# thalesfm/differentiable-renderer

Measured on AMD Instinct MI355X. Metric: Mray/s (fwd+bwd), Cornell 512x512 @64spp depth 8, higher is better.
Workload: dtype f32; 1 GPU; config 3: Cornell 512x512, 64 spp, depth 8, fwd + radiative backprop w.r.t. the albedos; scene 'cornell' (cornell box of render.cpp:26-59) 512x512, 64 spp per GPU, depth 8 (-b 8 -p 1), fwd + radiative-backprop gradients of 4 parameters; program=builtin, parallelism=1 GPU, gpu_max_hw_queues=4 (set by this script before the HIP runtime started)

## Files before the change

### differentiable-renderer_amd/csrc/drt_path.h

```cpp
#pragma once

#include "drt_kernels.h"

#define DRT_DRAW_TABLE (3 * DRT_MAX_DEPTH + 8)

struct PathArgs {
    int32_t W, H, spp;
    int32_t shard, n_shards, band;
    uint32_t Pb, p0, Sb, s0, spr, n_ranges, n_groups;
    int32_t min_bounces, depth_cap, cap_is_roulette, cap_draws;
    uint32_t rr_threshold, seed, rng_stream;
    uint32_t regen_min;
    uint32_t shade_min, descend_min;
    int32_t gimg_param;
    uint32_t gen_rows, gen_clog2;
    uint32_t hist_lds, hist_stride;
    uint32_t gimg_row, pad_gen;
    unsigned long long hist_ovf;
    double p_rr, inv_p_rr;
    double eye[3], fwd[3], right[3], up[3];
    double tan_half, aspect, inv_W, inv_H;
    float p_rr_f, inv_p_rr_f;
    float eye_f[3], fwd_f[3], right_f[3], up_f[3], cs_step_f, ct_step_f;
};

__device__ inline uint32_t path_global_pixel(const PathArgs& a, uint32_t lp)
{
    uint32_t ly = lp / (uint32_t)a.W, x = lp - ly * (uint32_t)a.W;
    uint32_t y = ly;
    if (a.n_shards > 1) {
        uint32_t b = ly / (uint32_t)a.band, r = ly - b * (uint32_t)a.band;
        y = (b * (uint32_t)a.n_shards + (uint32_t)a.shard) * (uint32_t)a.band + r;
    }
    return y * (uint32_t)a.W + x;
}

template <typename SG>
__device__ inline HitRec<float> path_closest_hit(const DevScene<float>* __restrict__ sc, const ProgRecs<SG::n>& recs, float4 ra, float2 rb)
{
    return closest_hit_prog<SG>(sc, recs, mk<float>(ra.x, ra.y, ra.z), mk<float>(ra.w, rb.x, rb.y));
}
template <typename SG>
__device__ inline HitRec<double> path_closest_hit(const DevScene<double>* __restrict__ sc, const ProgRecs<SG::n, double>& recs, double4 ra, double2 rb)
{
    if (SG::n > 0)
        return closest_hit_sig<SG, double>(recs, mk<double>(ra.x, ra.y, ra.z), mk<double>(ra.w, rb.x, rb.y));
    const double4 ra1[1] = {ra};
    const double2 rb1[1] = {rb};
    HitRec<double> h1[1];
    closest_hit_n<double, 1>(sc, sc->n_shapes, ra1, rb1, h1);
    return h1[0];
}

#define DRT_SIG_CORNELL                                                                                                   \
    ((unsigned long long)DRT_PK_SPHERE | (unsigned long long)DRT_PK_SPHERE << 3 | (unsigned long long)DRT_PK_AX << 6 |    \
     (unsigned long long)DRT_PK_PLANE << 9 | (unsigned long long)DRT_PK_AZ << 12 | (unsigned long long)DRT_PK_AZ << 15 |  \
     (unsigned long long)DRT_PK_AY << 18 | (unsigned long long)DRT_PK_AY << 21 | (unsigned long long)DRT_PK_SPHERE << 24)
#define DRT_NSIG_CORNELL 9
typedef KindSig<DRT_SIG_CORNELL, 0ull, 0ull, 0ull, DRT_NSIG_CORNELL> SigCornell;


template <typename R>
struct PathSceneLds {
    struct {
        int n_shapes, n_materials, n_emitters, n_params;
        DevShape<R> shapes[DRT_MAX_SHAPES];
        DevMaterial<R> materials[DRT_MAX_MATERIALS];
        int emitter_param[DRT_MAX_EMITTERS];
        int flat[DRT_MAX_SHAPES];
    } sc;
    R params[DRT_PATH_LDS_PARAMS * 3];
#ifdef DRT_USER_SHAPES
    R user_q[DRT_MAX_SHAPES][4];
#endif
};

template <typename R, bool ALL_LDS = false>
__device__ inline V3<R> load_param(const PathSceneLds<R>& lds, const R* __restrict__ params, int id)
{
    if (ALL_LDS || id < DRT_PATH_LDS_PARAMS)
        return mk<R>(lds.params[id * 3], lds.params[id * 3 + 1], lds.params[id * 3 + 2]);
    return mk<R>(params[id * 3], params[id * 3 + 1], params[id * 3 + 2]);
}

template <typename R>
__device__ inline void stage_path_scene(PathSceneLds<R>& lds, const DevScene<R>* __restrict__ sc, const R* __restrict__ params)
{
    const int ns = sc->n_shapes, nm = sc->n_materials, ne = sc->n_emitters;
    if (threadIdx.x < 4)
        reinterpret_cast<int*>(&lds.sc)[threadIdx.x] = reinterpret_cast<const int*>(sc)[threadIdx.x];
    {
        const int* src = reinterpret_cast<const int*>(sc->shapes);
        int* dst = reinterpret_cast<int*>(lds.sc.shapes);
        for (int i = threadIdx.x; i < ns * (int)(sizeof(DevShape<R>) / sizeof(int)); i += blockDim.x)
            dst[i] = src[i];
    }
    {
        const int* src = reinterpret_cast<const int*>(sc->materials);
        int* dst = reinterpret_cast<int*>(lds.sc.materials);
        for (int i = threadIdx.x; i < nm * (int)(sizeof(DevMaterial<R>) / sizeof(int)); i += blockDim.x)
            dst[i] = src[i];
    }
    for (int i = threadIdx.x; i < ne; i += blockDim.x)
        lds.sc.emitter_param[i] = sc->emitter_param[i];
    for (int i = threadIdx.x; i < ns; i += blockDim.x)
        lds.sc.flat[i] = sc->flat[i];
#ifdef DRT_USER_SHAPES
    for (int i = threadIdx.x; i < ns * 4; i += blockDim.x)
        lds.user_q[i >> 2][i & 3] = sc->user_q[i >> 2][i & 3];
#endif
    const int np = sc->n_params < DRT_PATH_LDS_PARAMS ? sc->n_params : DRT_PATH_LDS_PARAMS;
    for (int i = threadIdx.x; i < np * 3; i += blockDim.x)
        lds.params[i] = params[i];
    __syncthreads();
}


template <typename R>
struct TangentLds {
    R colnz[DRT_FAST_PARAMS][4];
    R invc[DRT_FAST_PARAMS][4];
    uint32_t inc[DRT_FAST_PARAMS][4];
};

template <typename R, typename SL>
__device__ inline void stage_tangents(TangentLds<R>& tl, const SL& lds)
{
    if (threadIdx.x < DRT_FAST_PARAMS) {
        const int p = threadIdx.x;
        const bool in = p < lds.sc.n_params;
        uint32_t zinc = 0, zbits = 0;
#pragma unroll
        for (int ch = 0; ch < 3; ++ch) {
            const R c = in ? lds.params[p * 3 + ch] : R(1);
            const bool zero = abs_r(c) < R(1e-18);
            tl.colnz[p][ch] = zero ? R(1) : c;
            tl.invc[p][ch] = zero ? R(0) : R(1) / c;
            zinc |= zero ? 1u << (8 * ch) : 0u;
            zbits |= zero ? 1u << ch : 0u;
        }
        tl.colnz[p][3] = R(0);
        tl.invc[p][3] = R(0);
        tl.inc[p][0] = p < 4 ? 1u << (8 * p) : 0u;
        tl.inc[p][1] = p >= 4 ? 1u << (8 * (p - 4)) : 0u;
        tl.inc[p][2] = zinc;
        tl.inc[p][3] = zbits;
    }
    __syncthreads();
}

template <typename R, int NP, int NC>
struct Tangents {
    uint32_t cnt[NC > 4 ? 2 : 1];
    uint32_t zc;
    R* acc;
    __device__ inline V3<R> acc_get(int p) const { return mk<R>(acc[(p * 3) * DRT_BLOCK], acc[(p * 3 + 1) * DRT_BLOCK], acc[(p * 3 + 2) * DRT_BLOCK]); }
    __device__ inline void acc_set(int p, V3<R> v) { acc[(p * 3) * DRT_BLOCK] = v.x; acc[(p * 3 + 1) * DRT_BLOCK] = v.y; acc[(p * 3 + 2) * DRT_BLOCK] = v.z; }
    __device__ inline void new_path() { cnt[0] = 0; if (NC > 4) cnt[NC > 4 ? 1 : 0] = 0; zc = 0; }
};

#define DRT_NP_ANY (-1)
#ifndef DRT_LOCKSTEP_MIN_BLOCKS
#define DRT_LOCKSTEP_MIN_BLOCKS 7
#endif
#ifndef DRT_LOCKSTEP_GEN_MIN_BLOCKS
#define DRT_LOCKSTEP_GEN_MIN_BLOCKS 6
#endif
#ifndef DRT_LOCKSTEP_SPEC_MIN_BLOCKS
#define DRT_LOCKSTEP_SPEC_MIN_BLOCKS 6
#endif
#ifndef DRT_REGEN_MIN_BLOCKS
#define DRT_REGEN_MIN_BLOCKS 5
#endif
#ifndef DRT_F64_MIN_BLOCKS
#define DRT_F64_MIN_BLOCKS 4
#endif
#ifndef DRT_GEN_TABLE
#define DRT_GEN_TABLE 408
#endif
template <bool B, typename X, typename Y> struct PickT { typedef X T; };
template <typename X, typename Y> struct PickT<false, X, Y> { typedef Y T; };
struct NoLds { int unused; };
template <typename R> struct GenAcc { typedef double T; };
#ifdef DRT_GEN_F32
template <> struct GenAcc<float> { typedef float T; };
#endif

template <typename R>
struct GenLds {
    R colnz[DRT_PATH_LDS_PARAMS][4];
    R invc[DRT_PATH_LDS_PARAMS][4];
};

template <typename R, typename SL>
__device__ inline void stage_gen(GenLds<R>& gl, const SL& lds, const DevScene<R>* __restrict__ sc)
{
    for (int p = threadIdx.x; p < DRT_PATH_LDS_PARAMS; p += blockDim.x) {
        const bool in = p < lds.sc.n_params;
        uint32_t zinc = 0, zbits = 0;
#pragma unroll
        for (int ch = 0; ch < 3; ++ch) {
            const R c = in ? lds.params[p * 3 + ch] : R(1);
            const bool zero = abs_r(c) < R(1e-18);
            gl.colnz[p][ch] = zero ? R(1) : c;
            gl.invc[p][ch] = zero ? R(0) : R(1) / c;
            zinc |= zero ? 1u << (8 * ch) : 0u;
            zbits |= zero ? 1u << ch : 0u;
        }
        const uint32_t slot = in ? (uint32_t)sc->grad_slot[p] : DRT_SLOT_NONE;
        gl.colnz[p][3] = pid_pack(R(0), zinc);
        gl.invc[p][3] = pid_pack(R(0), slot | zbits << 16);
    }
    __syncthreads();
}

template <typename R, int NC>
struct Tangents<R, DRT_NP_ANY, NC> {
    typedef typename GenAcc<R>::T GT;
    uint32_t cur;
    uint32_t zc;
    uint32_t nv;
    uint32_t* hist;
    uint32_t* hist_ovf;
    uint32_t hist_lds, hist_stride;
    const GenLds<R>* gl;
    GT* table;
    uint32_t clog2;
    R* acc;
    V3<R> gsum;
    uint32_t gimg_row;
    __device__ inline void new_path() { cur = 0xFFFFFFFFu; zc = 0; nv = 0; }
    __device__ inline void store_word(uint32_t w, uint32_t v)
    {
        if (w < hist_lds) hist[w * DRT_BLOCK] = v;
        else hist_ovf[(size_t)(w - hist_lds) * hist_stride] = v;
    }
    __device__ inline uint32_t load_word(uint32_t w) const
    {
        return w < hist_lds ? hist[w * DRT_BLOCK] : hist_ovf[(size_t)(w - hist_lds) * hist_stride];
    }
    template <bool UNIFORM>
    __device__ inline void push(bool live, uint32_t id)
    {
        const uint32_t shifted = (cur >> 8) | (id << 24);
        if (UNIFORM) {
            cur = shifted;
            ++nv;
            if ((nv & 3u) == 0u) {
                store_word((nv >> 2) - 1u, cur);
                cur = 0xFFFFFFFFu;
            }
        } else {
            cur = live ? shifted : cur;
            nv += live ? 1u : 0u;
            if (live && (nv & 3u) == 0u) {
                store_word((nv >> 2) - 1u, cur);
                cur = 0xFFFFFFFFu;
            }
        }
    }
    __device__ inline void add(uint32_t row, V3<R> v)
    {
        if constexpr (NC == 1) {
            const bool mine = row == gimg_row;
            gsum = mk<R>(gsum.x + (mine ? v.x : R(0)), gsum.y + (mine ? v.y : R(0)), gsum.z + (mine ? v.z : R(0)));
        }
        GT* t = table + ((row * 3u) << clog2);
        atomicAdd(t, (GT)v.x);
        atomicAdd(t + (1u << clog2), (GT)v.y);
        atomicAdd(t + (2u << clog2), (GT)v.z);
    }
    __device__ inline void add_word(uint32_t wd, V3<R> TgE, V3<R> U)
    {
#pragma unroll
        for (int b = 0; b < 4; ++b) {
            const uint32_t id = (wd >> (8 * b)) & 0xFFu;
            const bool valid = id != 0xFFu;
            if (wave_any(valid)) {
                if (valid) {
                    const R* rec = gl->invc[id];
                    const R ix = rec[0], iy = rec[1], iz = rec[2];
                    const uint32_t bits = pid_unpack(rec[3]);
                    const uint32_t row = bits & 0xFFFFu;
                    if (row != DRT_SLOT_NONE)
                        add(row, mk<R>((bits & 0x10000u) ? U.x : TgE.x * ix, (bits & 0x20000u) ? U.y : TgE.y * iy,
                                       (bits & 0x40000u) ? U.z : TgE.z * iz));
                }
            }
        }
    }
};

template <typename R>
struct GenBlock {
    GenLds<R> gl;
    typename GenAcc<R>::T table[DRT_BLOCK / DRT_WAVE][DRT_GEN_TABLE];
};
template <typename R>
__device__ inline void gen_zero(GenBlock<R>& gb)
{
    typedef typename GenAcc<R>::T GT;
    for (uint32_t i = threadIdx.x; i < (DRT_BLOCK / DRT_WAVE) * DRT_GEN_TABLE; i += DRT_BLOCK)
        (&gb.table[0][0])[i] = GT(0);
}
template <typename R, int NC, typename SL>
__device__ inline void gen_begin(GenBlock<R>& gb, const SL& lds, const DevScene<R>* __restrict__ sc, const PathArgs& a, uint32_t* hist,
                                 uint32_t* hist_ovf, Tangents<R, DRT_NP_ANY, NC>& tg)
{
    stage_gen(gb.gl, lds, sc);
    tg.gl = &gb.gl;
    tg.hist = hist + threadIdx.x;
    tg.hist_ovf = hist_ovf + (size_t)blockIdx.x * DRT_BLOCK + threadIdx.x;
    tg.gsum = mk<R>(R(0), R(0), R(0));
    tg.gimg_row = a.gimg_row;
    tg.hist_lds = a.hist_lds;
    tg.hist_stride = a.hist_stride;
    tg.clog2 = a.gen_clog2;
    tg.table = &gb.table[threadIdx.x / DRT_WAVE][threadIdx.x & ((1u << a.gen_clog2) - 1u)];
    tg.acc = nullptr;
    tg.new_path();
}
template <typename R>
__device__ inline void gen_finish(const GenBlock<R>& gb, const PathArgs& a, double* __restrict__ gpart)
{
    __syncthreads();
    const uint32_t copies = 1u << a.gen_clog2;
    for (uint32_t r = threadIdx.x; r < a.gen_rows; r += DRT_BLOCK) {
        double v = 0;
        for (int ww = 0; ww < DRT_BLOCK / DRT_WAVE; ++ww)
            for (uint32_t c = 0; c < copies; ++c)
                v += (double)gb.table[ww][(r << a.gen_clog2) + c];
        gpart[(size_t)blockIdx.x * a.gen_rows + r] = v;
    }
}

template <typename R, int NP, int NC, bool LOSS = false, typename SL = PathSceneLds<R>>
__device__ inline void add_emission(const SL& lds, const TangentLds<R>& tl, const R* __restrict__ params, uint32_t eid, R inv_pk,
                                    V3<R> T, V3<R> g, V3<R>& L, Tangents<R, NP, NC>& tg)
{
    const V3<R> E = load_param<R, (NP != 0)>(lds, params, (int)eid) * inv_pk;
    V3<R> Tr = T;
    if (NC > 0 || NP == DRT_NP_ANY)
        Tr = mk<R>((tg.zc & 0xFFu) ? R(0) : T.x, (tg.zc & 0xFF00u) ? R(0) : T.y, (tg.zc & 0xFF0000u) ? R(0) : T.z);
    L = L + Tr * E;
    if constexpr (NP == DRT_NP_ANY) {
        if (LOSS)
            g = mk<R>(R(2) * (L.x - g.x), R(2) * (L.y - g.y), R(2) * (L.z - g.z));
        const V3<R> gE = g * E;
        const uint32_t ebits = pid_unpack(tg.gl->invc[eid < DRT_PATH_LDS_PARAMS ? eid : 0][3]);
        if ((ebits & 0xFFFFu) != DRT_SLOT_NONE && eid < DRT_PATH_LDS_PARAMS)
            tg.add(ebits & 0xFFFFu, g * Tr * inv_pk);
        const V3<R> TgE = Tr * gE;
        const V3<R> U = mk<R>((tg.zc & 0xFFu) == 0x1u ? T.x * gE.x : R(0), (tg.zc & 0xFF00u) == 0x100u ? T.y * gE.y : R(0),
                              (tg.zc & 0xFF0000u) == 0x10000u ? T.z * gE.z : R(0));
        const uint32_t nw = tg.nv >> 2;
        for (uint32_t w = 0; wave_any(w < nw); ++w)
            tg.add_word(w < nw ? tg.load_word(w) : 0xFFFFFFFFu, TgE, U);
        tg.add_word(tg.cur, TgE, U);
    } else
    if constexpr (NP > 0) {
        if (NC > 0)
            asm volatile("" ::: "memory");
        if (LOSS)
            g = mk<R>(R(2) * (L.x - g.x), R(2) * (L.y - g.y), R(2) * (L.z - g.z));
        const V3<R> gE = g * E, gT = g * Tr * inv_pk;
#pragma unroll
        for (int p = 0; p < NP; ++p) {
            const bool own = eid == (uint32_t)p;
            const V3<R> ap = tg.acc_get(p);
            const V3<R> a0 = mk<R>(ap.x + (own ? gT.x : R(0)), ap.y + (own ? gT.y : R(0)), ap.z + (own ? gT.z : R(0)));
            if (p < NC) {
                const uint32_t n = (tg.cnt[p >> 2] >> (8 * (p & 3))) & 0xFFu;
                const R nf = (R)(int)n;
                V3<R> dT = mk<R>(Tr.x * (nf * tl.invc[p][0]), Tr.y * (nf * tl.invc[p][1]), Tr.z * (nf * tl.invc[p][2]));
                const uint32_t zb = __builtin_amdgcn_readfirstlane(tl.inc[p][3]);
                if (zb) {
                    const bool one = n == 1u;
                    if (zb & 1u) dT.x = (one && (tg.zc & 0xFFu) == 0x1u) ? T.x : R(0);
                    if (zb & 2u) dT.y = (one && (tg.zc & 0xFF00u) == 0x100u) ? T.y : R(0);
                    if (zb & 4u) dT.z = (one && (tg.zc & 0xFF0000u) == 0x10000u) ? T.z : R(0);
                }
                tg.acc_set(p, mk<R>(fma_r(dT.x, gE.x, a0.x), fma_r(dT.y, gE.y, a0.y), fma_r(dT.z, gE.z, a0.z)));
            } else
                tg.acc_set(p, a0);
        }
    }
}

template <typename R>
struct CameraLane {
    R cs0, ct0;
};

template <typename R>
struct PathVertex {
    V3<R> P, nrm, d;
    uint32_t ids;
    int material;
    bool hit, scattered;
};

template <typename R, bool SPEC, int NP, int NC, typename SG>
__device__ inline void path_bounce(const PathArgs& a, const PathSceneLds<R>& lds, const TangentLds<R>& tl, const DevScene<R>* __restrict__ sc,
                                   const R* __restrict__ params, const ProgRecs<SG::n, R>& recs, uint32_t key,
                                   R pk, R inv_pk, uint32_t n_theta, bool next_rr, bool next_cap, bool live, V3<R> g,
                                   typename Q4<R>::T& ra, typename Q2<R>::T& rb, V3<R>& T, V3<R>& L, Tangents<R, NP, NC>& tg,
                                   bool& alive, bool& capped, bool& on_light, uint32_t& light, PathVertex<R>* vo = nullptr,
                                   bool last = false, const float* __restrict__ seed_px = nullptr, const uint32_t* ih = nullptr)
{
    auto draw = [&](uint32_t n) { return ih ? drt_rng_combine(ih[n], key) : rng_draw(a.rng_stream, key, n); };
    const HitRec<R> h = path_closest_hit<SG>(sc, recs, ra, rb);
    const bool hit = live && h.prim >= 0;
    const int prim = h.prim >= 0 ? h.prim : 0;
    const V3<R> o = mk<R>(ra.x, ra.y, ra.z);
    const V3<R> d = mk<R>(ra.w, rb.x, rb.y);
    const V3<R> P = o + d * h.t;
    const DevShape<R>& sh = lds.sc.shapes[prim];
    const uint32_t ids = (uint32_t)sh.pad;
    const uint32_t cid = ids & 0xFFFFu, eid = ids >> 16;
    const bool has_bxdf = cid != DRT_ID_NONE, emits = hit && eid != DRT_ID_NONE;
    on_light = emits && !has_bxdf;
    light = eid;
    if (last && !vo) {
        if (wave_any(emits && has_bxdf)) {
            if (emits && has_bxdf) {
                if (NP != 0 && seed_px)
                    g = mk<R>((R)seed_px[0], (R)seed_px[1], (R)seed_px[2]);
                add_emission<R, NP, NC>(lds, tl, params, eid, inv_pk, T, g, L, tg);
            }
        }
        alive = false;
        capped = false;
        if (!a.cap_is_roulette) {
            const bool rr_kills = next_rr && draw(n_theta + 2) < a.rr_threshold;
            capped = hit && has_bxdf && !rr_kills;
        }
        return;
    }
    const V3<R> ctr = mk<R>(sh.p[0], sh.p[1], sh.p[2]);
    const V3<R> nsph = normalize(P - ctr);
    const bool is_plane = sh.type == DRT_SHAPE_PLANE;
    V3<R> nrm = mk<R>(is_plane ? ctr.x : nsph.x, is_plane ? ctr.y : nsph.y, is_plane ? ctr.z : nsph.z);
#ifdef DRT_USER_SHAPES
    if (sh.type >= DRT_SHAPE_USER) {
        const R p8[8] = {sh.p[0], sh.p[1], sh.p[2], sh.p[3], lds.user_q[prim][0], lds.user_q[prim][1], lds.user_q[prim][2], lds.user_q[prim][3]};
        nrm = user_normal<R>(sh.type - DRT_SHAPE_USER, p8, P);
    }
#endif
    if (vo) {
        vo->P = P; vo->nrm = nrm; vo->d = d;
        vo->ids = ids;
        vo->material = sh.material;
        vo->hit = hit;
        vo->scattered = hit && has_bxdf;
    }
    if (wave_any(emits && has_bxdf)) {
        if (emits && has_bxdf) {
            if (NP != 0 && seed_px)
                g = mk<R>((R)seed_px[0], (R)seed_px[1], (R)seed_px[2]);
            add_emission<R, NP, NC>(lds, tl, params, eid, inv_pk, T, g, L, tg);
        }
    }
    const DevMaterial<R>& m = lds.sc.materials[has_bxdf ? sh.material : 0];
    V3<R> wo;
    R q, bs;
    sample_bxdf<R, SPEC>(m, nrm, d, draw(n_theta), draw(n_theta + 1), wo, q, bs);
    const R c = dot(nrm, wo);
    const R mk_ = div_r(bs * c, q * pk);
    const bool rr_kills = next_rr && draw(n_theta + 2) < a.rr_threshold;
    alive = hit && has_bxdf && !next_cap && !rr_kills;
    capped = hit && has_bxdf && next_cap && !a.cap_is_roulette && !rr_kills;
    const int cidx = has_bxdf ? (int)cid : 0;
    V3<R> col;
    if constexpr (NP == DRT_NP_ANY) {
        const R* rec = tg.gl->colnz[cidx < DRT_PATH_LDS_PARAMS ? cidx : 0];
        col = mk<R>(rec[0], rec[1], rec[2]);
        tg.zc += alive ? pid_unpack(rec[3]) : 0u;
        if (ih)
            tg.template push<false>(alive, cid);
        else
            tg.template push<true>(live, alive ? cid : 0xFFu);
    } else
        col = NC > 0 ? mk<R>(tl.colnz[cidx][0], tl.colnz[cidx][1], tl.colnz[cidx][2]) : load_param<R, (NP > 0)>(lds, params, cidx);
    const V3<R> cmv = col * mk_;
    const V3<R> cm = mk<R>(alive ? cmv.x : R(1), alive ? cmv.y : R(1), alive ? cmv.z : R(1));
    if constexpr (NC > 0 && NP != DRT_NP_ANY) {
        tg.cnt[0] += alive ? tl.inc[cidx][0] : 0u;
        if (NC > 4)
            tg.cnt[NC > 4 ? 1 : 0] += alive ? tl.inc[cidx][1] : 0u;
        tg.zc += alive ? tl.inc[cidx][2] : 0u;
    }
    T = T * cm;
    const V3<R> no = P + wo * R(1e-3);
    ra.x = no.x; ra.y = no.y; ra.z = no.z; ra.w = wo.x;
    rb.x = wo.y; rb.y = wo.z;
}

#ifndef DRT_CAMERA_ARGS_F32
#define DRT_CAMERA_ARGS_F32 1
#endif
template <typename R, bool ARGS_F32 = (DRT_CAMERA_ARGS_F32 != 0)>
__device__ inline uint32_t path_camera(const PathArgs& a, const CameraLane<R>& cl, uint32_t gpix, uint32_t px, uint32_t py, uint32_t sl,
                                       typename Q4<R>::T& ra, typename Q2<R>::T& rb)
{
    const uint64_t path = (uint64_t)gpix * (uint64_t)a.spp + (uint64_t)(a.s0 + sl);
    const uint32_t key = (uint32_t)path;
    if (sizeof(R) == 4) {
        const float cs_step = ARGS_F32 ? a.cs_step_f : (float)(2. * a.aspect * a.tan_half * a.inv_W);
        const float ct_step = ARGS_F32 ? a.ct_step_f : (float)(2. * a.tan_half * a.inv_H);
        const V3<float> eye = ARGS_F32 ? mk<float>(a.eye_f[0], a.eye_f[1], a.eye_f[2]) : mk<float>((float)a.eye[0], (float)a.eye[1], (float)a.eye[2]);
        const V3<float> fw = ARGS_F32 ? mk<float>(a.fwd_f[0], a.fwd_f[1], a.fwd_f[2]) : mk<float>((float)a.fwd[0], (float)a.fwd[1], (float)a.fwd[2]);
        const V3<float> rt = ARGS_F32 ? mk<float>(a.right_f[0], a.right_f[1], a.right_f[2]) : mk<float>((float)a.right[0], (float)a.right[1], (float)a.right[2]);
        const V3<float> upv = ARGS_F32 ? mk<float>(a.up_f[0], a.up_f[1], a.up_f[2]) : mk<float>((float)a.up[0], (float)a.up[1], (float)a.up[2]);
        const float cs = fmaf(u01(0.f, rng_draw(a.rng_stream, key, 0)), cs_step, (float)cl.cs0);
        const float ct = fmaf(u01(0.f, rng_draw(a.rng_stream, key, 1)), ct_step, (float)cl.ct0);
        const V3<float> dir = mk<float>(fw.x + cs * rt.x - ct * upv.x, fw.y + cs * rt.y - ct * upv.y, fw.z + cs * rt.z - ct * upv.z);
        const V3<float> dn = normalize(dir);
        ra.x = (R)eye.x; ra.y = (R)eye.y; ra.z = (R)eye.z; ra.w = (R)dn.x;
        rb.x = (R)dn.y; rb.y = (R)dn.z;
    } else {
        const double u1 = (double)rng_draw(a.rng_stream, key, 0) / DRT_RAND_MAX_D;
        const double u2 = (double)rng_draw(a.rng_stream, key, 1) / DRT_RAND_MAX_D;
        const double s = ((double)px + u1) / (double)a.W;
        const double t = ((double)py + u2) / (double)a.H;
        const double cs = (2. * s - 1.) * a.aspect * a.tan_half;
        const double ct = (2. * t - 1.) * a.tan_half;
        double dx = a.fwd[0] + cs * a.right[0] - ct * a.up[0];
        double dy = a.fwd[1] + cs * a.right[1] - ct * a.up[1];
        double dz = a.fwd[2] + cs * a.right[2] - ct * a.up[2];
        const double inv = 1.0 / sqrt(dx * dx + dy * dy + dz * dz);
        ra.x = (R)a.eye[0]; ra.y = (R)a.eye[1]; ra.z = (R)a.eye[2]; ra.w = (R)(dx * inv);
        rb.x = (R)(dy * inv); rb.y = (R)(dz * inv);
    }
    return key;
}
template <typename R>
__device__ inline uint32_t path_camera(const PathArgs& a, const CameraLane<R>& cl, uint32_t gpix, uint32_t sl,
                                       typename Q4<R>::T& ra, typename Q2<R>::T& rb)
{
    uint32_t px = 0, py = 0;
    if (sizeof(R) != 4) {
        py = gpix / (uint32_t)a.W;
        px = gpix - py * (uint32_t)a.W;
    }
    return path_camera<R, false>(a, cl, gpix, px, py, sl, ra, rb);
}

#ifndef DRT_LEAN_MAX_SHAPES
#ifdef DRT_USER_SHAPES
#define DRT_LEAN_MAX_SHAPES (-1)
#else
#define DRT_LEAN_MAX_SHAPES 10
#endif
#endif
template <size_t RB, bool SPEC, int NP, int NSG, bool REGEN>
constexpr int path_min_blocks()
{
    if (RB == 4 && NP <= 4) {
        if (!REGEN)
            return SPEC ? ((NP == DRT_NP_ANY || NSG > DRT_LEAN_MAX_SHAPES) ? 5 : DRT_LOCKSTEP_SPEC_MIN_BLOCKS)
                        : (NP == DRT_NP_ANY ? DRT_LOCKSTEP_GEN_MIN_BLOCKS : (NSG <= DRT_LEAN_MAX_SHAPES ? DRT_LOCKSTEP_MIN_BLOCKS : DRT_LOCKSTEP_GEN_MIN_BLOCKS));
        return (NP == DRT_NP_ANY && NSG == 0) ? 4
                                              : (SPEC ? 5 : DRT_REGEN_MIN_BLOCKS);
    }
    return (RB == 8 && NP <= 4 && !REGEN && !SPEC) ? DRT_F64_MIN_BLOCKS : 1;
}

template <typename R, bool SPEC, int NP, int NC, typename SG, bool REGEN = false, bool LOSS = false>
__global__ void __launch_bounds__(DRT_BLOCK, (path_min_blocks<sizeof(R), SPEC, NP, SG::n, REGEN>()))
k_path(PathArgs a, const DevScene<R>* __restrict__ sc, const R* __restrict__ params, const float* __restrict__ adjoint,
       double* __restrict__ gpart, double* __restrict__ fpart, uint32_t* __restrict__ counts,
       unsigned long long* __restrict__ total, double* __restrict__ gimg_part)
{
    if (total && blockIdx.x == 0 && threadIdx.x < 8)
        total[threadIdx.x] = 0;
    typedef typename Q4<R>::T R4;
    typedef typename Q2<R>::T R2;
    __shared__ PathSceneLds<R> lds;
    __shared__ double s_red[REGEN ? 1 : DRT_BLOCK / DRT_WAVE][DRT_FAST_PARAMS * 3];
    __shared__ TangentLds<R> s_tl;
    constexpr bool GEN = NP == DRT_NP_ANY;
    __shared__ typename PickT<GEN, GenBlock<R>, NoLds>::T s_gen;
    extern __shared__ uint32_t s_hist[];
    if constexpr (GEN)
        gen_zero(s_gen);
    stage_path_scene(lds, sc, params);
    const TangentLds<R>& tl = s_tl;
    if (NC > 0 && !GEN)
        stage_tangents(s_tl, lds);

    const uint32_t lane = threadIdx.x & (DRT_WAVE - 1);
    const uint32_t w = grid_wave();
    const uint32_t range = w / a.n_groups, group = w - range * a.n_groups;
    const uint32_t lp = group * DRT_WAVE + lane;
    const bool have = range < a.n_ranges && lp < a.Pb;
    const uint32_t s_begin = range * a.spr;
    const uint32_t s_end = s_begin + a.spr < a.Sb ? s_begin + a.spr : a.Sb;

    Tangents<R, NP, NC> tg;
    __shared__ R s_acc[NP > 0 ? NP * 3 : 1][DRT_BLOCK];
    tg.acc = &s_acc[0][threadIdx.x];
    if constexpr (GEN)
        gen_begin(s_gen, lds, sc, a, s_hist, reinterpret_cast<uint32_t*>(a.hist_ovf), tg);
    else {
#pragma unroll
        for (int p = 0; p < NP; ++p)
            tg.acc_set(p, mk<R>(R(0), R(0), R(0)));
    }
    double fx = 0, fy = 0, fz = 0;
    uint32_t n_seg = 0, n_capped = 0;

    uint32_t gpix = 0, px = 0, py = 0;
    V3<R> g = mk<R>(R(1), R(1), R(1));
    if (have) {
        gpix = path_global_pixel(a, a.p0 + lp);
        py = gpix / (uint32_t)a.W;
        px = gpix - py * (uint32_t)a.W;
        if (NP != 0 && adjoint)
            g = mk<R>((R)adjoint[(size_t)gpix * 3], (R)adjoint[(size_t)gpix * 3 + 1], (R)adjoint[(size_t)gpix * 3 + 2]);
    }
    CameraLane<R> cl;
    cl.cs0 = (R)((2. * (double)px * a.inv_W - 1.) * a.aspect * a.tan_half);
    cl.ct0 = (R)((2. * (double)py * a.inv_H - 1.) * a.tan_half);
    constexpr bool ARGS_F32 = sizeof(R) == 4 && !REGEN && DRT_CAMERA_ARGS_F32 != 0 && SG::n <= DRT_LEAN_MAX_SHAPES;
    const R pk_rr = ARGS_F32 ? (R)a.p_rr_f : (R)a.p_rr, inv_p_rr = ARGS_F32 ? (R)a.inv_p_rr_f : (R)a.inv_p_rr;
    ProgRecs<SG::n, R> recs;
    __shared__ typename PickT<(SG::n == 0), ProgLds, NoLds>::T s_prog;
    recs.lds = reinterpret_cast<const ProgLds*>(&s_prog);
    if (SG::n > 0)
        recs.template load<SG>(sc);
    if constexpr (sizeof(R) == 4 && SG::n == 0) {
        const DevScene<float>* scf = reinterpret_cast<const DevScene<float>*>(sc);
        if (threadIdx.x < DRT_PROG_SORTED_MAX) {
            s_prog.rec[threadIdx.x] = *reinterpret_cast<const float4*>(scf->sorted[threadIdx.x]);
            s_prog.shape[threadIdx.x] = scf->sorted_shape[threadIdx.x];
        }
        if (threadIdx.x < 8)
            s_prog.kind_begin[threadIdx.x] = scf->kind_begin[threadIdx.x];
        __syncthreads();
    }

    if (range < a.n_ranges && !REGEN) {
    for (uint32_t sl = s_begin; sl < s_end; ++sl) {
        R4 ra;
        R2 rb;
        const uint32_t key = path_camera<R, ARGS_F32>(a, cl, gpix, px, py, sl, ra, rb);
        bool live = have && a.depth_cap > 0 && !(a.min_bounces <= 0 && rng_draw(a.rng_stream, key, 2) < a.rr_threshold);
        V3<R> T = mk<R>(R(1), R(1), R(1)), L = mk<R>(R(0), R(0), R(0));
        uint32_t end_ids = DRT_ID_NONE;
        R end_inv_pk = R(1);
        if (NC > 0 || GEN)
            tg.new_path();
        for (int kk = 0; kk < a.depth_cap; ++kk) {
            const uint32_t n_live = (uint32_t)__popcll(wave_ballot(live));
            if (n_live == 0)
                break;
            n_seg += n_live;
            const R pk = kk >= a.min_bounces ? pk_rr : R(1);
            const R inv_pk = kk >= a.min_bounces ? inv_p_rr : R(1);
            const uint32_t n_theta = draw_offset(kk, 0, a.min_bounces) + camera_draw_base(a.min_bounces);
            const bool next_rr = (kk + 1) >= a.min_bounces;
            const bool next_cap = (kk + 1) >= a.depth_cap;
            bool alive, capped, on_light;
            uint32_t light;
            path_bounce<R, SPEC, NP, NC, SG>(a, lds, tl, sc, params, recs, key, pk, inv_pk, n_theta, next_rr, next_cap, live, g,
                                                    ra, rb, T, L, tg, alive, capped, on_light, light, nullptr, next_cap);
            end_ids = on_light ? light : end_ids;
            end_inv_pk = on_light ? inv_pk : end_inv_pk;
            if (next_cap && !a.cap_is_roulette)
                n_capped += (uint32_t)__popcll(wave_ballot(capped));
            live = alive;
        }
        if (wave_any(end_ids != DRT_ID_NONE)) {
            if (end_ids != DRT_ID_NONE)
                add_emission<R, NP, NC, LOSS>(lds, tl, params, end_ids, end_inv_pk, T, g, L, tg);
        }
        fx += (double)L.x; fy += (double)L.y; fz += (double)L.z;
    }
    }
    __shared__ R s_pcs[REGEN ? DRT_BLOCK : 1], s_pct[REGEN ? DRT_BLOCK : 1];
    __shared__ uint32_t s_pgpix[REGEN ? DRT_BLOCK : 1];
    __shared__ double s_film[REGEN ? 3 : 1][REGEN ? DRT_BLOCK : 1];
    __shared__ uint32_t s_ih[REGEN ? DRT_DRAW_TABLE : 1];
    if (REGEN) {
        for (uint32_t n = threadIdx.x; n < DRT_DRAW_TABLE; n += DRT_BLOCK)
            s_ih[REGEN ? n : 0] = drt_rng_index_hash(a.rng_stream, n);
        s_pcs[threadIdx.x] = cl.cs0;
        s_pct[threadIdx.x] = cl.ct0;
        s_pgpix[threadIdx.x] = have ? gpix : 0xFFFFFFFFu;
        s_film[0][threadIdx.x] = 0.0; s_film[REGEN ? 1 : 0][threadIdx.x] = 0.0; s_film[REGEN ? 2 : 0][threadIdx.x] = 0.0;
        __syncthreads();
    }
    if (range < a.n_ranges && REGEN) {
        const uint32_t wbase = threadIdx.x & ~(uint32_t)(DRT_WAVE - 1);
        const uint32_t n_items = DRT_WAVE * (s_end - s_begin);
        uint32_t n_next = 0;
        uint32_t key = 0, pix = wbase, pgpix = 0;
        int kk = 0;
        bool live = false;
        R4 ra;
        R2 rb;
        ra.x = ra.y = ra.z = ra.w = R(0);
        rb.x = rb.y = R(0);
        V3<R> T = mk<R>(R(1), R(1), R(1)), L = mk<R>(R(0), R(0), R(0));
        if (NC > 0 || GEN)
            tg.new_path();
        const int first_rr = a.min_bounces > 1 ? a.min_bounces : 1;
        for (;;) {
            const uint64_t idle_mask = wave_ballot(!live);
            const uint32_t n_idle = (uint32_t)__popcll(idle_mask), n_run = DRT_WAVE - n_idle;
            if (n_next < n_items && (n_idle >= a.regen_min || n_idle >= n_run)) {
                const uint32_t n = n_next + __builtin_amdgcn_mbcnt_hi((uint32_t)(idle_mask >> 32), __builtin_amdgcn_mbcnt_lo((uint32_t)idle_mask, 0u));
                if (!live && n < n_items) {
                    pix = wbase + (n & (DRT_WAVE - 1));
                    const uint32_t gp = s_pgpix[pix];
                    if (gp != 0xFFFFFFFFu) {
                        pgpix = gp;
                        CameraLane<R> pc;
                        pc.cs0 = s_pcs[pix];
                        pc.ct0 = s_pct[pix];
                        key = path_camera<R>(a, pc, gp, s_begin + (n >> 6), ra, rb);
                        kk = 0;
                        live = a.depth_cap > 0 && !(a.min_bounces <= 0 && rng_draw(a.rng_stream, key, 2) < a.rr_threshold);
                        T = mk<R>(R(1), R(1), R(1));
                        L = mk<R>(R(0), R(0), R(0));
                        if (NC > 0 || GEN)
                            tg.new_path();
                    }
                }
                n_next += n_idle < n_items - n_next ? n_idle : n_items - n_next;
            }
            const uint32_t n_live = (uint32_t)__popcll(wave_ballot(live));
            if (n_live == 0) {
                if (n_next >= n_items)
                    break;
                continue;
            }
            n_seg += n_live;
            const bool rr_here = kk >= a.min_bounces;
            const R pk = rr_here ? pk_rr : R(1);
            const R inv_pk = rr_here ? inv_p_rr : R(1);
            const int rr_draws = kk - first_rr + 1;
            const uint32_t n_theta = 2u * (uint32_t)kk + (uint32_t)(rr_draws > 0 ? rr_draws : 0) + camera_draw_base(a.min_bounces);
            const bool next_rr = (kk + 1) >= a.min_bounces;
            const bool next_cap = (kk + 1) >= a.depth_cap;
            bool alive, capped, on_light;
            uint32_t light;
            V3<R> gp3 = mk<R>(R(1), R(1), R(1));
            const float* seed_px = (NP != 0 && adjoint) ? adjoint + (size_t)pgpix * 3 : (const float*)nullptr;
            path_bounce<R, SPEC, NP, NC, SG>(a, lds, tl, sc, params, recs, key, pk, inv_pk, n_theta, next_rr, next_cap, live, gp3,
                                                    ra, rb, T, L, tg, alive, capped, on_light, light, nullptr, false, seed_px, s_ih);
            if (!a.cap_is_roulette)
                n_capped += (uint32_t)__popcll(wave_ballot(capped));
            const bool ended = live && !alive;
            if (wave_any(ended)) {
                if (ended) {
                    if (on_light) {
                        if (seed_px)
                            gp3 = mk<R>((R)seed_px[0], (R)seed_px[1], (R)seed_px[2]);
                        add_emission<R, NP, NC, LOSS>(lds, tl, params, light, inv_pk, T, gp3, L, tg);
                    }
                    if (L.x != R(0) || L.y != R(0) || L.z != R(0)) {
                        atomicAdd(&s_film[0][pix], (double)L.x);
                        atomicAdd(&s_film[REGEN ? 1 : 0][pix], (double)L.y);
                        atomicAdd(&s_film[REGEN ? 2 : 0][pix], (double)L.z);
                    }
                }
            }
            live = alive;
            ++kk;
        }
    }
    if (REGEN) {
        __syncthreads();
        fx = s_film[0][threadIdx.x]; fy = s_film[REGEN ? 1 : 0][threadIdx.x]; fz = s_film[REGEN ? 2 : 0][threadIdx.x];
    }

    if (range < a.n_ranges) {
        if (fpart && have) {
            double* f = fpart + ((size_t)range * 3) * a.Pb + lp;
            f[0] = fx; f[(size_t)a.Pb] = fy; f[(size_t)a.Pb * 2] = fz;
        }
        if constexpr (GEN && NC == 1) if (gimg_part && have) {
            double* f = gimg_part + ((size_t)range * 3) * a.Pb + lp;
            f[0] = (double)tg.gsum.x; f[(size_t)a.Pb] = (double)tg.gsum.y; f[(size_t)a.Pb * 2] = (double)tg.gsum.z;
        }
        if constexpr (NP > 0) if (gimg_part && have) {
            const V3<R> v = tg.acc_get(a.gimg_param > 0 && a.gimg_param < NP ? a.gimg_param : 0);
            double* f = gimg_part + ((size_t)range * 3) * a.Pb + lp;
            f[0] = (double)v.x; f[(size_t)a.Pb] = (double)v.y; f[(size_t)a.Pb * 2] = (double)v.z;
        }
        if (lane == 0) {
            counts[w] = n_seg;
            counts[(size_t)a.n_groups * a.n_ranges + w] = n_capped;
        }
    }
    if constexpr (GEN)
        gen_finish(s_gen, a, gpart);
    else
    if (NP > 0) {
        const int wv = threadIdx.x / DRT_WAVE;
        double (*red)[DRT_FAST_PARAMS * 3] = s_red;
        if (REGEN) {
            __syncthreads();
            red = reinterpret_cast<double (*)[DRT_FAST_PARAMS * 3]>(&s_film[0][0]);
        }
#pragma unroll
        for (int r = 0; r < NP * 3; ++r) {
            double v = (double)tg.acc[r * DRT_BLOCK];
#pragma unroll
            for (int o2 = DRT_WAVE / 2; o2 > 0; o2 >>= 1)
                v += __shfl_down(v, o2);
            if (lane == 0)
                red[wv][r] = v;
        }
        __syncthreads();
        if (threadIdx.x < DRT_FAST_PARAMS * 3) {
            double v = 0;
            if ((int)threadIdx.x < NP * 3)
                for (int ww = 0; ww < DRT_BLOCK / DRT_WAVE; ++ww)
                    v += red[ww][threadIdx.x];
            gpart[(size_t)blockIdx.x * (DRT_FAST_PARAMS * 3) + threadIdx.x] = v;
        }
    }
}

template <typename R, bool SPEC, typename SG>
__device__ inline void unbiased_walk(const PathArgs& a, const PathSceneLds<R>& lds, const TangentLds<R>& tl, const DevScene<R>* __restrict__ sc,
                                     const R* __restrict__ params, const ProgRecs<SG::n, R>& recs, uint32_t key,
                                     R pk_rr, R inv_p_rr, bool live, typename Q4<R>::T ra, typename Q2<R>::T rb, int kk,
                                     uint32_t& nd, uint32_t& n_seg, uint32_t& n_capped, V3<R>& L, PathVertex<R>& first, bool& any_vertex)
{
    V3<R> T = mk<R>(R(1), R(1), R(1));
    L = mk<R>(R(0), R(0), R(0));
    any_vertex = false;
    Tangents<R, 0, 0> none;
    const V3<R> g1 = mk<R>(R(1), R(1), R(1));
    for (;;) {
        const uint32_t n_live = (uint32_t)__popcll(wave_ballot(live));
        if (n_live == 0)
            break;
        n_seg += n_live;
        const bool rr_here = kk >= a.min_bounces;
        const R pk = rr_here ? pk_rr : R(1), inv_pk = rr_here ? inv_p_rr : R(1);
        const bool next_rr = (kk + 1) >= a.min_bounces, next_cap = (kk + 1) >= a.depth_cap;
        bool alive, capped, on_light;
        uint32_t light;
        PathVertex<R> v;
        path_bounce<R, SPEC, 0, 0, SG>(a, lds, tl, sc, params, recs, key, pk, inv_pk, nd, next_rr, next_cap, live, g1, ra, rb, T, L,
                                              none, alive, capped, on_light, light, &v);
        const uint32_t rr_drawn = (next_rr && (!next_cap || a.cap_draws)) ? 1u : 0u;
        if (live) {
            if (!any_vertex && v.hit) {
                first = v;
                any_vertex = true;
            }
            nd += v.scattered ? 2u + rr_drawn : (v.hit ? rr_drawn : 0u);
        }
        if (wave_any(live && on_light)) {
            if (live && on_light)
                add_emission<R, 0, 0>(lds, tl, params, light, inv_pk, T, g1, L, none);
        }
        if (!a.cap_is_roulette)
            n_capped += (uint32_t)__popcll(wave_ballot(live && capped));
        live = alive;
        ++kk;
    }
}

#ifndef DRT_UNBIASED_MIN_BLOCKS
#define DRT_UNBIASED_MIN_BLOCKS 4
#endif
template <typename R, bool SPEC, int NP, typename SG>
__global__ void __launch_bounds__(DRT_BLOCK, (sizeof(R) == 4 ? DRT_UNBIASED_MIN_BLOCKS : 1))
k_path_unbiased(PathArgs a, const DevScene<R>* __restrict__ sc, const R* __restrict__ params, const float* __restrict__ adjoint,
                double* __restrict__ gpart, double* __restrict__ fpart, uint32_t* __restrict__ counts,
                unsigned long long* __restrict__ total)
{
    if (total && blockIdx.x == 0 && threadIdx.x < 8)
        total[threadIdx.x] = 0;
    typedef typename Q4<R>::T R4;
    typedef typename Q2<R>::T R2;
    __shared__ PathSceneLds<R> lds;
    __shared__ double s_red[DRT_BLOCK / DRT_WAVE][DRT_FAST_PARAMS * 3];
    constexpr bool GEN = NP == DRT_NP_ANY;
    __shared__ typename PickT<GEN, GenBlock<R>, NoLds>::T s_gen;
    if constexpr (GEN)
        gen_zero(s_gen);
    stage_path_scene(lds, sc, params);
    const TangentLds<R>& tl = *reinterpret_cast<const TangentLds<R>*>(&lds);
    Tangents<R, GEN ? DRT_NP_ANY : 0, 0> gt;
    if constexpr (GEN)
        gen_begin(s_gen, lds, sc, a, (uint32_t*)nullptr, (uint32_t*)nullptr, gt);

    const uint32_t lane = threadIdx.x & (DRT_WAVE - 1);
    const uint32_t w = grid_wave();
    const uint32_t range = w / a.n_groups, group = w - range * a.n_groups;
    const uint32_t lp = group * DRT_WAVE + lane;
    const bool have = range < a.n_ranges && lp < a.Pb;
    const uint32_t s_begin = range * a.spr;
    const uint32_t s_end = s_begin + a.spr < a.Sb ? s_begin + a.spr : a.Sb;

    V3<R> acc[NP > 0 ? NP : 1];
#pragma unroll
    for (int p = 0; p < NP; ++p)
        acc[p] = mk<R>(R(0), R(0), R(0));
    double fx = 0, fy = 0, fz = 0;
    uint32_t n_seg = 0, n_capped = 0;
    uint32_t gpix = 0, px = 0, py = 0;
    V3<R> g0 = mk<R>(R(1), R(1), R(1));
    if (have) {
        gpix = path_global_pixel(a, a.p0 + lp);
        py = gpix / (uint32_t)a.W;
        px = gpix - py * (uint32_t)a.W;
        if (adjoint)
            g0 = mk<R>((R)adjoint[(size_t)gpix * 3], (R)adjoint[(size_t)gpix * 3 + 1], (R)adjoint[(size_t)gpix * 3 + 2]);
    }
    CameraLane<R> cl;
    cl.cs0 = (R)((2. * (double)px * a.inv_W - 1.) * a.aspect * a.tan_half);
    cl.ct0 = (R)((2. * (double)py * a.inv_H - 1.) * a.tan_half);
    constexpr bool ARGS_F32 = sizeof(R) == 4 && DRT_CAMERA_ARGS_F32 != 0 && SG::n <= DRT_LEAN_MAX_SHAPES;
    const R pk_rr = ARGS_F32 ? (R)a.p_rr_f : (R)a.p_rr, inv_p_rr = ARGS_F32 ? (R)a.inv_p_rr_f : (R)a.inv_p_rr;
    ProgRecs<SG::n, R> recs;
    __shared__ ProgLds s_prog;
    recs.lds = &s_prog;
    if (SG::n > 0)
        recs.template load<SG>(sc);
    if (sizeof(R) == 4 && SG::n == 0) {
        const DevScene<float>* scf = reinterpret_cast<const DevScene<float>*>(sc);
        if (threadIdx.x < DRT_PROG_SORTED_MAX) {
            s_prog.rec[threadIdx.x] = *reinterpret_cast<const float4*>(scf->sorted[threadIdx.x]);
            s_prog.shape[threadIdx.x] = scf->sorted_shape[threadIdx.x];
        }
        if (threadIdx.x < 8)
            s_prog.kind_begin[threadIdx.x] = scf->kind_begin[threadIdx.x];
        __syncthreads();
    }
    auto rr_drawn = [&](int d) { return d >= a.min_bounces && (d < a.depth_cap || a.cap_draws != 0); };

    if (range < a.n_ranges) {
        for (uint32_t sl = s_begin; sl < s_end; ++sl) {
            R4 ra;
            R2 rb;
            const uint32_t key = path_camera<R, ARGS_F32>(a, cl, gpix, px, py, sl, ra, rb);
            uint32_t nd = 2;
            bool live = have && a.depth_cap > 0;
            if (rr_drawn(0)) {
                live = live && !(rng_draw(a.rng_stream, key, nd) < a.rr_threshold);
                ++nd;
            }
            V3<R> L0;
            PathVertex<R> cur;
            bool in_chain;
            unbiased_walk<R, SPEC, SG>(a, lds, tl, sc, params, recs, key, pk_rr, inv_p_rr, live, ra, rb, 0, nd, n_seg, n_capped, L0,
                                              cur, in_chain);
            fx += (double)L0.x; fy += (double)L0.y; fz += (double)L0.z;
            in_chain = in_chain && have;
            int cdepth = 0;
            V3<R> g = g0;
            while (wave_any(in_chain)) {
                V3<R> gq = mk<R>(R(0), R(0), R(0)), fcol = gq;
                R bs = R(0);
                bool go = false;
                R4 sa = ra;
                R2 sb = rb;
                uint32_t cid = DRT_ID_NONE;
                if (in_chain) {
                    const R inv_pk = cdepth >= a.min_bounces ? inv_p_rr : R(1);
                    const V3<R> g1 = g * inv_pk;
                    const uint32_t eid = cur.ids >> 16;
                    cid = cur.ids & 0xFFFFu;
                    if constexpr (GEN) {
                        if (eid < DRT_PATH_LDS_PARAMS) {
                            const uint32_t row = pid_unpack(gt.gl->invc[eid][3]) & 0xFFFFu;
                            if (row != DRT_SLOT_NONE)
                                gt.add(row, g1);
                        }
                    }
#pragma unroll
                    for (int p = 0; p < NP; ++p) {
                        const bool own = eid == (uint32_t)p;
                        acc[p] = mk<R>(acc[p].x + (own ? g1.x : R(0)), acc[p].y + (own ? g1.y : R(0)), acc[p].z + (own ? g1.z : R(0)));
                    }
                    if (cid == DRT_ID_NONE) {
                        in_chain = false;
                    } else {
                        const DevMaterial<R>& m = lds.sc.materials[cur.material];
                        V3<R> wo;
                        R q;
                        sample_bxdf<R, SPEC>(m, cur.nrm, cur.d, rng_draw(a.rng_stream, key, nd), rng_draw(a.rng_stream, key, nd + 1), wo, q, bs);
                        nd += 2;
                        const R c = dot(cur.nrm, wo);
                        gq = g1 * div_r(c, q);
                        fcol = load_param<R, true>(lds, params, (int)cid) * bs;
                        go = (cdepth + 1) < a.depth_cap;
                        if (rr_drawn(cdepth + 1)) {
                            go = go && !(rng_draw(a.rng_stream, key, nd) < a.rr_threshold);
                            ++nd;
                        }
                        const V3<R> no = cur.P + wo * R(1e-3);
                        sa.x = no.x; sa.y = no.y; sa.z = no.z; sa.w = wo.x;
                        sb.x = wo.y; sb.y = wo.z;
                    }
                }
                V3<R> Ls;
                PathVertex<R> nxt;
                bool any_vertex;
                unbiased_walk<R, SPEC, SG>(a, lds, tl, sc, params, recs, key, pk_rr, inv_p_rr, in_chain && go, sa, sb, cdepth + 1, nd,
                                                  n_seg, n_capped, Ls, nxt, any_vertex);
                if (in_chain) {
                    const V3<R> df = Ls * gq * bs;
                    if constexpr (GEN) {
                        if (cid < DRT_PATH_LDS_PARAMS) {
                            const uint32_t row = pid_unpack(gt.gl->invc[cid][3]) & 0xFFFFu;
                            if (row != DRT_SLOT_NONE)
                                gt.add(row, df);
                        }
                    }
#pragma unroll
                    for (int p = 0; p < NP; ++p) {
                        const bool own = cid == (uint32_t)p;
                        acc[p] = mk<R>(acc[p].x + (own ? df.x : R(0)), acc[p].y + (own ? df.y : R(0)), acc[p].z + (own ? df.z : R(0)));
                    }
                    if (!any_vertex) {
                        in_chain = false;
                    } else {
                        g = fcol * gq;
                        cur = nxt;
                        ++cdepth;
                    }
                }
            }
        }
        if (fpart && have) {
            double* f = fpart + ((size_t)range * 3) * a.Pb + lp;
            f[0] = fx; f[(size_t)a.Pb] = fy; f[(size_t)a.Pb * 2] = fz;
        }
        if (lane == 0) {
            counts[w] = n_seg;
            counts[(size_t)a.n_groups * a.n_ranges + w] = n_capped;
        }
    }
    if constexpr (GEN)
        gen_finish(s_gen, a, gpart);
    else
    {
        const int wv = threadIdx.x / DRT_WAVE;
#pragma unroll
        for (int r = 0; r < NP * 3; ++r) {
            const V3<R> v3 = acc[r / 3];
            double v = (double)(r % 3 == 0 ? v3.x : (r % 3 == 1 ? v3.y : v3.z));
#pragma unroll
            for (int o2 = DRT_WAVE / 2; o2 > 0; o2 >>= 1)
                v += __shfl_down(v, o2);
            if (lane == 0)
                s_red[wv][r] = v;
        }
        __syncthreads();
        if (threadIdx.x < DRT_FAST_PARAMS * 3) {
            double v = 0;
            if ((int)threadIdx.x < NP * 3)
                for (int ww = 0; ww < DRT_BLOCK / DRT_WAVE; ++ww)
                    v += s_red[ww][threadIdx.x];
            gpart[(size_t)blockIdx.x * (DRT_FAST_PARAMS * 3) + threadIdx.x] = v;
        }
    }
}

__global__ void __launch_bounds__(DRT_BLOCK)
k_film_parts(const double* __restrict__ fpart, uint32_t n_ranges, uint32_t Pb, uint32_t p0, double* __restrict__ film)
{
    const uint32_t stride = gridDim.x * blockDim.x;
    for (uint32_t j = blockIdx.x * blockDim.x + threadIdx.x; j < Pb; j += stride) {
        double r = 0, g = 0, b = 0;
        for (uint32_t q = 0; q < n_ranges; ++q) {
            const double* f = fpart + ((size_t)q * 3) * Pb + j;
            r += f[0]; g += f[(size_t)Pb]; b += f[(size_t)Pb * 2];
        }
        double* f = film + (size_t)(p0 + j) * 3;
        f[0] += r; f[1] += g; f[2] += b;
    }
}

__global__ void __launch_bounds__(DRT_BLOCK)
k_path_finish(PathArgs a, const double* __restrict__ fpart, float* __restrict__ out, uint32_t film_blocks,
              const double* __restrict__ gpart, int n_blocks, int n_rows, int row_stride, double* __restrict__ grad, uint32_t grad_words,
              const uint32_t* __restrict__ counts, uint32_t n_waves, unsigned long long* __restrict__ total, uint32_t count_rows = 2,
              const unsigned short* __restrict__ slot_map = nullptr)
{
    __shared__ double red[DRT_BLOCK];
    if (blockIdx.x < film_blocks) {
        const uint32_t stride = film_blocks * DRT_BLOCK;
        const double inv = 1.0 / (double)a.spp;
        for (uint32_t j = blockIdx.x * DRT_BLOCK + threadIdx.x; j < a.Pb; j += stride) {
            double r = 0, g = 0, b = 0;
            for (uint32_t q = 0; q < a.n_ranges; ++q) {
                const double* f = fpart + ((size_t)q * 3) * a.Pb + j;
                r += f[0]; g += f[(size_t)a.Pb]; b += f[(size_t)a.Pb * 2];
            }
            const uint32_t gp = path_global_pixel(a, a.p0 + j);
            drt_f3 px;
            px.x = (float)(r * inv); px.y = (float)(g * inv); px.z = (float)(b * inv);
            *reinterpret_cast<drt_f3_u*>(out + (size_t)gp * 3) = px;
        }
        return;
    }
    if (blockIdx.x < film_blocks + grad_words) {
        const int p = (int)(blockIdx.x - film_blocks);
        int src = p;
        if (slot_map) {
            const int slot = slot_map[p / 3];
            src = slot == (int)DRT_SLOT_NONE ? n_rows : slot * 3 + p % 3;
        }
        double v = 0;
        if (src < n_rows)
            for (int b = threadIdx.x; b < n_blocks; b += DRT_BLOCK)
                v += gpart[(size_t)b * row_stride + src];
        red[threadIdx.x] = v;
        __syncthreads();
        for (int off = DRT_BLOCK / 2; off > 0; off >>= 1) {
            if ((int)threadIdx.x < off)
                red[threadIdx.x] += red[threadIdx.x + off];
            __syncthreads();
        }
        if (threadIdx.x == 0)
            grad[p] = red[0];
        return;
    }
    {
        const uint32_t nb = gridDim.x - film_blocks - grad_words, me = blockIdx.x - film_blocks - grad_words;
        unsigned long long seg = 0, cap = 0, wlk = 0;
        for (uint32_t i = me * DRT_BLOCK + threadIdx.x; i < n_waves; i += nb * DRT_BLOCK) {
            seg += counts[i];
            cap += counts[(size_t)n_waves + i];
            if (count_rows > 2)
                wlk += counts[(size_t)n_waves * 2 + i];
        }
        for (int off = DRT_WAVE / 2; off > 0; off >>= 1) {
            seg += __shfl_down(seg, off);
            cap += __shfl_down(cap, off);
            wlk += __shfl_down(wlk, off);
        }
        if ((threadIdx.x & (DRT_WAVE - 1)) == 0) {
            if (seg) atomicAdd(total, seg);
            if (cap) atomicAdd(total + 3, cap);
            if (wlk) atomicAdd(total + 5, wlk);
        }
    }
}
```

Baseline: 195,400 Mray/s.

## Defer per-parameter gradient scaling to range end via raw emission sums

Adds a SUMS mode for non-regenerating, non-loss path kernels that accumulates per-parameter sums of count-weighted throughput times emission, without multiplying by the pixel gradient or the inverse albedo at each emission. The factors g*(1/c) are applied once per lane after the sample range in finish_range_sums, and direct emitter-parameter contributions are pre-scaled by c so the final division cancels. This moves multiplications out of the per-emission hot path and adds two small LDS tables. The factoring relies on g being constant across the range, which holds only when no per-sample seed gradient is reloaded.

```diff
diff --git a/differentiable-renderer_amd/csrc/drt_path.h b/differentiable-renderer_amd/csrc/drt_path.h
--- a/differentiable-renderer_amd/csrc/drt_path.h
+++ b/differentiable-renderer_amd/csrc/drt_path.h
@@ -121,9 +121,11 @@
     R colnz[DRT_FAST_PARAMS][4];
     R invc[DRT_FAST_PARAMS][4];
     uint32_t inc[DRT_FAST_PARAMS][4];
+    R fin[DRT_FAST_PARAMS][4];
+    R escale[DRT_FAST_PARAMS][4];
 };
 
-template <typename R, typename SL>
+template <int NC = DRT_FAST_PARAMS, typename R, typename SL>
 __device__ inline void stage_tangents(TangentLds<R>& tl, const SL& lds)
 {
     if (threadIdx.x < DRT_FAST_PARAMS) {
@@ -136,11 +138,15 @@
             const bool zero = abs_r(c) < R(1e-18);
             tl.colnz[p][ch] = zero ? R(1) : c;
             tl.invc[p][ch] = zero ? R(0) : R(1) / c;
+            tl.fin[p][ch] = (p >= NC || zero) ? R(1) : R(1) / c;
+            tl.escale[p][ch] = (p >= NC || zero) ? R(1) : c;
             zinc |= zero ? 1u << (8 * ch) : 0u;
             zbits |= zero ? 1u << ch : 0u;
         }
         tl.colnz[p][3] = R(0);
         tl.invc[p][3] = R(0);
+        tl.fin[p][3] = R(0);
+        tl.escale[p][3] = R(0);
         tl.inc[p][0] = p < 4 ? 1u << (8 * p) : 0u;
         tl.inc[p][1] = p >= 4 ? 1u << (8 * (p - 4)) : 0u;
         tl.inc[p][2] = zinc;
@@ -334,7 +340,7 @@
     }
 }
 
-template <typename R, int NP, int NC, bool LOSS = false, typename SL = PathSceneLds<R>>
+template <typename R, int NP, int NC, bool LOSS = false, bool SUMS = false, typename SL = PathSceneLds<R>>
 __device__ inline void add_emission(const SL& lds, const TangentLds<R>& tl, const R* __restrict__ params, uint32_t eid, R inv_pk,
                                     V3<R> T, V3<R> g, V3<R>& L, Tangents<R, NP, NC>& tg)
 {
@@ -343,6 +349,33 @@
     if (NC > 0 || NP == DRT_NP_ANY)
         Tr = mk<R>((tg.zc & 0xFFu) ? R(0) : T.x, (tg.zc & 0xFF00u) ? R(0) : T.y, (tg.zc & 0xFF0000u) ? R(0) : T.z);
     L = L + Tr * E;
+    if constexpr (SUMS && NP > 0 && NP != DRT_NP_ANY && !LOSS) {
+        if (NC > 0)
+            asm volatile("" ::: "memory");
+#pragma unroll
+        for (int p = 0; p < NC; ++p) {
+            const uint32_t n = (tg.cnt[p >> 2] >> (8 * (p & 3))) & 0xFFu;
+            const R nf = (R)(int)n;
+            const V3<R> a0 = tg.acc_get(p), nE = E * nf;
+            V3<R> s = mk<R>(fma_r(Tr.x, nE.x, a0.x), fma_r(Tr.y, nE.y, a0.y), fma_r(Tr.z, nE.z, a0.z));
+            const uint32_t zb = __builtin_amdgcn_readfirstlane(tl.inc[p][3]);
+            if (zb) {
+                const bool one = n == 1u;
+                if (zb & 1u) s.x = a0.x + ((one && (tg.zc & 0xFFu) == 0x1u) ? T.x * E.x : R(0));
+                if (zb & 2u) s.y = a0.y + ((one && (tg.zc & 0xFF00u) == 0x100u) ? T.y * E.y : R(0));
+                if (zb & 4u) s.z = a0.z + ((one && (tg.zc & 0xFF0000u) == 0x10000u) ? T.z * E.z : R(0));
+            }
+            tg.acc_set(p, s);
+        }
+        if (eid < (uint32_t)NP) {
+            const V3<R> s = mk<R>(tl.escale[eid][0], tl.escale[eid][1], tl.escale[eid][2]);
+            const V3<R> Tp = Tr * inv_pk;
+            R* r = tg.acc + (eid * 3) * DRT_BLOCK;
+            r[0] = fma_r(Tp.x, s.x, r[0]);
+            r[DRT_BLOCK] = fma_r(Tp.y, s.y, r[DRT_BLOCK]);
+            r[2 * DRT_BLOCK] = fma_r(Tp.z, s.z, r[2 * DRT_BLOCK]);
+        }
+    } else
     if constexpr (NP == DRT_NP_ANY) {
         if (LOSS)
             g = mk<R>(R(2) * (L.x - g.x), R(2) * (L.y - g.y), R(2) * (L.z - g.z));
@@ -387,6 +420,24 @@
     }
 }
 
+#ifndef DRT_PATH_RANGE_SUMS
+#define DRT_PATH_RANGE_SUMS 1
+#endif
+template <int NP, int NC, bool REGEN, bool LOSS>
+constexpr bool range_sums()
+{
+    return DRT_PATH_RANGE_SUMS != 0 && NP > 0 && NP != DRT_NP_ANY && NC > 0 && !REGEN && !LOSS;
+}
+template <typename R, int NP, int NC>
+__device__ inline void finish_range_sums(const TangentLds<R>& tl, V3<R> g, Tangents<R, NP, NC>& tg)
+{
+#pragma unroll
+    for (int p = 0; p < NP; ++p) {
+        const V3<R> s = tg.acc_get(p);
+        tg.acc_set(p, mk<R>(s.x * (g.x * tl.fin[p][0]), s.y * (g.y * tl.fin[p][1]), s.z * (g.z * tl.fin[p][2])));
+    }
+}
+
 template <typename R>
 struct CameraLane {
     R cs0, ct0;
@@ -400,7 +451,7 @@
     bool hit, scattered;
 };
 
-template <typename R, bool SPEC, int NP, int NC, typename SG>
+template <typename R, bool SPEC, int NP, int NC, typename SG, bool SUMS = false>
 __device__ inline void path_bounce(const PathArgs& a, const PathSceneLds<R>& lds, const TangentLds<R>& tl, const DevScene<R>* __restrict__ sc,
                                    const R* __restrict__ params, const ProgRecs<SG::n, R>& recs, uint32_t key,
                                    R pk, R inv_pk, uint32_t n_theta, bool next_rr, bool next_cap, bool live, V3<R> g,
@@ -426,7 +477,7 @@
             if (emits && has_bxdf) {
                 if (NP != 0 && seed_px)
                     g = mk<R>((R)seed_px[0], (R)seed_px[1], (R)seed_px[2]);
-                add_emission<R, NP, NC>(lds, tl, params, eid, inv_pk, T, g, L, tg);
+                add_emission<R, NP, NC, false, SUMS>(lds, tl, params, eid, inv_pk, T, g, L, tg);
             }
         }
         alive = false;
@@ -458,7 +509,7 @@
         if (emits && has_bxdf) {
             if (NP != 0 && seed_px)
                 g = mk<R>((R)seed_px[0], (R)seed_px[1], (R)seed_px[2]);
-            add_emission<R, NP, NC>(lds, tl, params, eid, inv_pk, T, g, L, tg);
+            add_emission<R, NP, NC, false, SUMS>(lds, tl, params, eid, inv_pk, T, g, L, tg);
         }
     }
     const DevMaterial<R>& m = lds.sc.materials[has_bxdf ? sh.material : 0];
@@ -587,7 +638,8 @@
     stage_path_scene(lds, sc, params);
     const TangentLds<R>& tl = s_tl;
     if (NC > 0 && !GEN)
-        stage_tangents(s_tl, lds);
+        stage_tangents<NC>(s_tl, lds);
+    constexpr bool SUMS = range_sums<NP, NC, REGEN, LOSS>();
 
     const uint32_t lane = threadIdx.x & (DRT_WAVE - 1);
     const uint32_t w = grid_wave();
@@ -663,8 +715,8 @@
             const bool next_cap = (kk + 1) >= a.depth_cap;
             bool alive, capped, on_light;
             uint32_t light;
-            path_bounce<R, SPEC, NP, NC, SG>(a, lds, tl, sc, params, recs, key, pk, inv_pk, n_theta, next_rr, next_cap, live, g,
-                                                    ra, rb, T, L, tg, alive, capped, on_light, light, nullptr, next_cap);
+            path_bounce<R, SPEC, NP, NC, SG, SUMS>(a, lds, tl, sc, params, recs, key, pk, inv_pk, n_theta, next_rr, next_cap, live, g,
+                                                   ra, rb, T, L, tg, alive, capped, on_light, light, nullptr, next_cap);
             end_ids = on_light ? light : end_ids;
             end_inv_pk = on_light ? inv_pk : end_inv_pk;
             if (next_cap && !a.cap_is_roulette)
@@ -673,10 +725,12 @@
         }
         if (wave_any(end_ids != DRT_ID_NONE)) {
             if (end_ids != DRT_ID_NONE)
-                add_emission<R, NP, NC, LOSS>(lds, tl, params, end_ids, end_inv_pk, T, g, L, tg);
+                add_emission<R, NP, NC, LOSS, SUMS>(lds, tl, params, end_ids, end_inv_pk, T, g, L, tg);
         }
         fx += (double)L.x; fy += (double)L.y; fz += (double)L.z;
     }
+    if constexpr (SUMS)
+        finish_range_sums<R, NP>(tl, g, tg);
     }
     __shared__ R s_pcs[REGEN ? DRT_BLOCK : 1], s_pct[REGEN ? DRT_BLOCK : 1];
     __shared__ uint32_t s_pgpix[REGEN ? DRT_BLOCK : 1];
```

Result: faster. 198,100 Mray/s, median of 6 (+1.4%).
